# BerserkerMother/Video-Summarization

Measured on AMD Instinct MI355X. Metric: frames/sec scored (whole node), synthetic [B,T=1024,D=1024], higher is better.
Workload: dtype f32; 1 GPU; configs[2]: B=64 videos x T=1024 frames x D=1024 per GPU, scorer cfg M-A (heads 4, d_model 256, layers 4), logits + hidden state; global_batch=64, parallelism=videos sharded over 1 GPU(s), no all_gather of scores

## Files before the change

video-summarization_amd/csrc/vs_attention.hip:

```cpp
#include "vs_device.h"
#include "vs_kernels.h"

namespace {

template <int DH, int NKB, bool VARLEN = false>
__global__ __launch_bounds__(256, 2) void attn_fwd(
    const float *__restrict__ Q, const float *__restrict__ Kg, const float *__restrict__ Vg,
    const uint8_t *__restrict__ mask, float *__restrict__ out, int H, int T, float scale_log2e, int BH,
    const int *__restrict__ cu = nullptr, const int2 *__restrict__ work = nullptr, int Mtot = 0) {
    constexpr int KT = 32 * NKB, LD = DH + 4, NJ = DH / 8, ND = DH / 32;
    constexpr int F4 = KT * DH / 4 / 256;
    __shared__ __attribute__((aligned(16))) float Ks[KT * LD];
    __shared__ __attribute__((aligned(16))) float Vs[KT * LD];
    __shared__ float mb[KT];

    const int tid = threadIdx.x, lane = tid & 63, wave = tid >> 6;
    const int r = lane & 31, h = lane >> 5;
    int b, head, qt;
    size_t base, orow0;
    if constexpr (VARLEN) {
        const int2 wk = work[blockIdx.x];
        b = wk.x; qt = wk.y; head = blockIdx.y;
        const int c0 = cu[b];
        T = cu[b + 1] - c0;
// ... 750 lines not shown
        gload_m(KAHEAD);
        asm volatile("s_waitcnt vmcnt(0)" ::: "memory");
    } else {
#pragma unroll
        for (int u = 0; u < KAHEAD; ++u) {
            gload_k(u); gload_m(u);
            if (u < VAHEAD) gload_v(u);
#pragma unroll
            for (int i = 0; i < KPT; ++i) stage_k1(i, u % NBUF);
            if (u < VAHEAD) {
#pragma unroll
                for (int e = 0; e < 4; ++e) stage_v1(e, u % NBUF);
            }
            stage_m(u % NMB);
        }
        gload_k(KAHEAD); gload_m(KAHEAD); gload_v(VAHEAD);
    }
    __syncthreads();
    f32x16 sa[2], sb[2];
#pragma unroll
    for (int n = 0; n < 2; ++n)
#pragma unroll
        for (int t = 0; t < 16; ++t) { sa[n][t] = 0.f; sb[n][t] = 0.f; }
#pragma unroll
    for (int ks = 0; ks < NS; ++ks)
#pragma unroll
        for (int n = 0; n < 2; ++n) {
            u32x4 ka[NP];
            k_frag(0, ks, n, ka);
            static_for<NPROD>([&](auto prc) { mma_prod(prc, ka, qreg[ks], sa[n]); });
        }

    constexpr float CMARGIN = PREC == 2 ? -8.0f : 6.0f;
    (void)CMARGIN;
    u32x4 pf[2][2][NP];
    f16x2 pmaxh = {(_Float16)0.f, (_Float16)0.f};
    float cb_a = 0.f, cb_b = 0.f;
    auto rebase = [&](f32x16 (&sv)[2], float &cb, bool raise) __attribute__((always_inline)) {
        float mx = __builtin_fmaxf(__builtin_fmaxf(sv[0][0], sv[0][1]), sv[1][0]);
        mx = __builtin_fmaxf(mx, sv[1][1]);
#pragma unroll
        for (int t = 2; t < 16; t += 2) {
            mx = __builtin_fmaxf(__builtin_fmaxf(mx, sv[0][t]), sv[0][t + 1]);
            mx = __builtin_fmaxf(__builtin_fmaxf(mx, sv[1][t]), sv[1][t + 1]);
        }
        const float raw = pair_max(mx) + cb;
        float c_new = m_run;
        if ((raise || m_run == NEG_INF) && raw + CMARGIN > m_run) {
            const float cl = __builtin_fminf(__builtin_fmaxf(raw + CMARGIN, -32768.f), 32768.f);
            const unsigned b = __builtin_bit_cast(unsigned, cl);
            constexpr unsigned LOW = PREC == 2 ? 0x1FFFu : 0xFFFFu;
            c_new = __builtin_bit_cast(float, (cl >= 0.f ? b + LOW : b) & ~LOW);
            if (PREC == 1 && __builtin_fabsf(cl) >= 8192.f) c_new = __builtin_bit_cast(float, (b + 0x8000u) & ~LOW);
            if (PREC == 2 && __builtin_fabsf(c_new) < 0.0001220703125f) c_new = cl > 0.f ? 0.0001220703125f : 0.f;
        }
        const float u_new = (c_new == NEG_INF) ? 0.f : c_new;
        const float shift = cb - u_new;
        const float alpha = __builtin_amdgcn_exp2f(m_run - u_new);
#pragma unroll
        for (int n = 0; n < 2; ++n)
#pragma unroll
            for (int t = 0; t < 16; ++t) sv[n][t] += shift;
#pragma unroll
        for (int d = 0; d <= ND; ++d)
#pragma unroll
            for (int t = 0; t < 16; ++t) o[d][t] *= alpha;
        m_run = c_new;
        cb = u_new;
        unsigned pl[NP];
        pack(-u_new, 0.f, pl);
        nbias = h == 0 ? pl[0] : 0u;
    };
    auto p_pair = [&](auto kc, f32x16 (&sv)[2]) __attribute__((always_inline)) {
        constexpr int k = decltype(kc)::value, n = k / 8, ks = (k / 4) % 2, j = k % 4;
        unsigned pl[NP];
        pack(__builtin_amdgcn_exp2f(sv[n][8 * ks + 2 * j]), __builtin_amdgcn_exp2f(sv[n][8 * ks + 2 * j + 1]), pl);
#pragma unroll
        for (int p = 0; p < NP; ++p) pf[n][ks][p][j] = pl[p];
        if constexpr (PREC == 2) pmaxh = __builtin_elementwise_max(pmaxh, __builtin_bit_cast(f16x2, pl[0]));
    };
    float sm_mx = 0.f;
    f32x2 sm_mm = {0.f, 0.f};
    auto sm_unit_max = [&](auto uc, f32x16 (&sv)[2]) __attribute__((always_inline)) {
        constexpr int U = decltype(uc)::value;
        constexpr float THR = 8.0f;
        if constexpr (U == 0) {
            sm_mx = __builtin_fmaxf(__builtin_fmaxf(sv[0][0], sv[0][1]), sv[1][0]);
            sm_mx = __builtin_fmaxf(sm_mx, sv[1][1]);
        }
        if constexpr (U < 4) {
            constexpr int t0 = U == 0 ? 2 : 4 * U;
#pragma unroll
            for (int t = t0; t < 4 * U + 4; t += 2) {
                sm_mx = __builtin_fmaxf(__builtin_fmaxf(sm_mx, sv[0][t]), sv[0][t + 1]);
                sm_mx = __builtin_fmaxf(__builtin_fmaxf(sm_mx, sv[1][t]), sv[1][t + 1]);
            }
        }
        if constexpr (U == 4) {
            const float mx = pair_max(sm_mx);
            const bool raise = mx > m_run + THR || (m_run == NEG_INF && mx != NEG_INF);
            if (__builtin_expect(__any(raise), 0)) {
                const float m_new = raise ? mx : m_run;
                const float u_new = (m_new == NEG_INF) ? 0.f : m_new;
                const float alpha = __builtin_amdgcn_exp2f(m_run - u_new);
#pragma unroll
                for (int d = 0; d <= ND; ++d)
#pragma unroll
                    for (int t = 0; t < 16; ++t) o[d][t] *= alpha;
                m_run = m_new;
            }
            const float m_use = (m_run == NEG_INF) ? 0.f : m_run;
            sm_mm[0] = m_use; sm_mm[1] = m_use;
        }
        if constexpr (U >= 5 && U < 21) {
            constexpr int k = U - 5, n = k / 8, ks = (k / 4) % 2, j = k % 4;
            const f32x2 sx = {sv[n][8 * ks + 2 * j], sv[n][8 * ks + 2 * j + 1]};
            const f32x2 dv = sx - sm_mm;
            unsigned pl[NP];
            pack(__builtin_amdgcn_exp2f(dv[0]), __builtin_amdgcn_exp2f(dv[1]), pl);
#pragma unroll
            for (int p = 0; p < NP; ++p) pf[n][ks][p][j] = pl[p];
        }
    };
    auto sm_unit = [&](auto uc, f32x16 (&sv)[2], float &cb) __attribute__((always_inline)) {
        constexpr int U = decltype(uc)::value;
        if constexpr (!FOLD) { sm_unit_max(uc, sv); return; }
        if constexpr (U == 0) {
            const float u_run = (m_run == NEG_INF) ? 0.f : m_run;
            if (__builtin_expect(__any(cb != u_run || m_run == NEG_INF), 0)) rebase(sv, cb, false);
        }
        if constexpr (U >= 1 && U < 17) p_pair(std::integral_constant<int, U - 1>{}, sv);
        if constexpr (U == 17) {
            unsigned acc = 0u;
            bool hit;
            if constexpr (PREC == 2) {
                acc = __builtin_bit_cast(unsigned, pmaxh);
                hit = (acc & 0xFFFFu) >= 0x7800u || (acc >> 16) >= 0x7800u;
                pmaxh = f16x2{(_Float16)0.f, (_Float16)0.f};
            } else {
#pragma unroll
                for (int n = 0; n < 2; ++n)
#pragma unroll
                    for (int ks = 0; ks < 2; ++ks) acc |= (pf[n][ks][0][0] | pf[n][ks][0][1]) | (pf[n][ks][0][2] | pf[n][ks][0][3]);
                hit = (acc & 0x40004000u) != 0u;
            }
            if (__builtin_expect(__any(hit), 0)) {
                const unsigned hbit = hit ? 1u : 0u;
                auto pr = __builtin_amdgcn_permlane32_swap(hbit, hbit, false, false);
                rebase(sv, cb, (((unsigned)pr[0] | (unsigned)pr[1]) & 1u) != 0u);
                static_for<16>([&](auto kc) { p_pair(kc, sv); });
                if constexpr (PREC == 2) pmaxh = f16x2{(_Float16)0.f, (_Float16)0.f};
            }
        }
    };
    constexpr int NU = FOLD ? 18 : 21;
    constexpr bool FULLPF = PREC == 1 && DH <= 64;
    constexpr int NKF = FULLPF ? NS * 2 : 2, NVF = FULLPF ? 4 * ND : 2;
    constexpr int NBIAS = FOLD ? 2 : 0;
    constexpr int NSLOT_A = 2 * NS * NPROD + NBIAS, RA = (NU + NSLOT_A - 1) / NSLOT_A;
    constexpr int NSLOT_B = 4 * (ND * NPROD + NP);
    constexpr int NITEM = KPT + 4 + 2, SB = NSLOT_B / NITEM > 0 ? NSLOT_B / NITEM : 1;

    u32x4 abl_frag = {0u, 0u, 0u, 0u};
    if constexpr ((ABL & 16) != 0) abl_frag = *(const u32x4 *)&Kb[0][0][r * LDK + 8 * h];
    auto iteration = [&](int t, f32x16 (&s_in)[2], float &cb_in, f32x16 (&s_out)[2], float &cb_out) __attribute__((always_inline)) {
        const int cur = (ABL & 4) ? 0 : t % NBUF, nxt = (ABL & 4) ? 0 : (t + 1) % NBUF;
        if (mask != nullptr || (t + 1) * KT > T) {
            const float *mp = mb[t % NMB];
#pragma unroll
            for (int n = 0; n < 2; ++n)
#pragma unroll
                for (int g = 0; g < 4; ++g) {
                    const f32x4 bv = *(const f32x4 *)&mp[32 * n + 8 * g + 4 * h];
#pragma unroll
                    for (int e = 0; e < 4; ++e) s_in[n][4 * g + e] += bv[e];
                }
        }
        cb_out = (m_run == NEG_INF) ? 0.f : m_run;
        const u32x4 nb = {nbias, 0u, 0u, 0u};
        const f32x16 zero16 = {0.f, 0.f, 0.f, 0.f, 0.f, 0.f, 0.f, 0.f, 0.f, 0.f, 0.f, 0.f, 0.f, 0.f, 0.f, 0.f};
        u32x4 ka[NKF][NP], va[NVF][NP];
        if constexpr ((ABL & 16) != 0) {
#pragma unroll
            for (int g = 0; g < NKF; ++g)
#pragma unroll
                for (int p = 0; p < NP; ++p) ka[g][p] = abl_frag;
#pragma unroll
            for (int g = 0; g < NVF; ++g)
#pragma unroll
                for (int p = 0; p < NP; ++p) va[g][p] = abl_frag;
        } else
        if constexpr (FULLPF) {
#pragma unroll
            for (int g = 0; g < NS * 2; ++g) k_frag(nxt, g % NS, g / NS, ka[g]);
        } else {
            k_frag(nxt, 0, 0, ka[0]);
        }
        __builtin_amdgcn_sched_barrier(0);
        static_for<NSLOT_A>([&](auto ic) {
            constexpr int i = decltype(ic)::value, PERN = NS * NPROD, n = i < NBIAS ? i : (i - NBIAS) / PERN,
                          w = i < NBIAS ? 0 : 1 + (i - NBIAS) % PERN;
            if constexpr (w == 0) {
                s_out[n] = mma(ones_u, nb, zero16);
            } else {
                constexpr int ks = (w - 1) / NPROD, pr = (w - 1) % NPROD, g = n * NS + ks;
                if constexpr (!FOLD && w == 1) s_out[n] = zero16;
                if constexpr (!(ABL & 16) && !FULLPF && pr == 0 && g + 1 < NS * 2) k_frag(nxt, (g + 1) % NS, (g + 1) / NS, ka[(g + 1) & 1]);
                mma_prod(std::integral_constant<int, pr>{}, ka[FULLPF ? g : (g & 1)], qreg[ks], s_out[n]);
            }
            if constexpr (!(ABL & 16) && FULLPF && i >= NBIAS && i - NBIAS < NVF) {
                constexpr int f = i - NBIAS;
                v_frag(cur, f / ND / 2, (f / ND) % 2, f % ND, va[f]);
            }
            static_for<RA>([&](auto rc) {
                constexpr int U = i * RA + decltype(rc)::value;
                if constexpr (U < NU && !(ABL & 8)) sm_unit(std::integral_constant<int, U>{}, s_in, cb_in);
            });
            __builtin_amdgcn_sched_barrier(0);
        });
        lap(1);
        if constexpr (DMA) asm volatile("s_waitcnt vmcnt(0)" ::: "memory");
        if constexpr (STAG && !(ABL & 2)) { __syncthreads(); lap(3); }
        if constexpr (!FULLPF && !(ABL & 16)) v_frag(cur, 0, 0, 0, va[0]);
        __builtin_amdgcn_sched_barrier(0);
        static_for<NSLOT_B>([&](auto ic) {
            constexpr int i = decltype(ic)::value;
            constexpr int PER = ND * NPROD + NP;
            constexpr int g = i / PER, w = i % PER, n = g / 2, ks = g % 2;
            if constexpr (w < ND * NPROD) {
                constexpr int d = w / NPROD, pr = w % NPROD, f = g * ND + d;
                if constexpr (!(ABL & 16) && !FULLPF && pr == 0 && f + 1 < 4 * ND)
                    v_frag(cur, (f + 1) / ND / 2, ((f + 1) / ND) % 2, (f + 1) % ND, va[(f + 1) & 1]);
                mma_prod(std::integral_constant<int, pr>{}, va[FULLPF ? f : (f & 1)], pf[n][ks], o[d]);
            } else {
                constexpr int p = NP - 1 - (w - ND * NPROD);
                o[ND] = mma(ones_u, pf[n][ks][p], o[ND]);
            }
            if constexpr (DMA) {
                if constexpr (!(ABL & 1) && i == 0) dma_issue(t + KAHEAD, t + VAHEAD, true, true);
                if constexpr (!(ABL & 1) && i == 4) { stage_m((t + KAHEAD) % NMB); gload_m(t + KAHEAD + 1); }
            } else
            if constexpr (!(ABL & 1) && i % SB == SB - 1 && i / SB < NITEM) {
                constexpr int item = i / SB;
                if constexpr (item < KPT) stage_k1(item, (t + KAHEAD) % NBUF);
                else if constexpr (item < KPT + 4) stage_v1(item - KPT, (t + VAHEAD) % NBUF);
                else if constexpr (item == KPT + 4) { stage_m((t + KAHEAD) % NMB); }
                else { gload_k(t + KAHEAD + 1); gload_m(t + KAHEAD + 1); gload_v(t + VAHEAD + 1); }
            }
            __builtin_amdgcn_sched_barrier(0);
        });
        lap(2);
        if constexpr (!(ABL & 2)) __syncthreads();
        lap(3);
    };

    lap(0);
    const bool late = STAG && __builtin_amdgcn_readfirstlane(wave) >= NW / 2;
    if (late) __syncthreads();
    int t = 0;
    for (; t + 1 < ntiles; t += 2) {
        iteration(t, sa, cb_a, sb, cb_b);
        iteration(t + 1, sb, cb_b, sa, cb_a);
    }
    if (t < ntiles) iteration(t, sa, cb_a, sb, cb_b);
    if (STAG && !late) __syncthreads();

    const int q = q0 + r;
    if (q < T) {
        const float inv = 1.0f / o[ND][0];
        float *op = out + (orow0 + q) * (H * DH) + head * DH;
        h16 *op16 = (h16 *)out + (orow0 + q) * (H * DH) + head * DH;
#pragma unroll
        for (int d = 0; d < ND; ++d)
#pragma unroll
            for (int g = 0; g < 4; ++g) {
                f32x4 v;
#pragma unroll
                for (int e = 0; e < 4; ++e) v[e] = o[d][4 * g + e] * inv;
                if constexpr (IO16) {
                    u32x2 u; u[0] = pack_bf16(v[0], v[1]); u[1] = pack_bf16(v[2], v[3]);
                    *(u32x2 *)(op16 + 32 * d + 8 * g + 4 * h) = u;
                } else
                *(f32x4 *)(op + 32 * d + 8 * g + 4 * h) = v;
            }
    }
    if constexpr (DIAG != 0) {
        asm volatile("s_waitcnt vmcnt(0)" ::: "memory");
        lap(7);
        dg[8] = tl - tbeg; dg[10] = __builtin_amdgcn_s_memrealtime(); dg[11] = (unsigned long long)ntiles;
        if (diag != nullptr && lane == 0) {
            unsigned long long *o_ = diag + ((size_t)blockIdx.x * NW + wave) * 16;
#pragma unroll
            for (int i = 0; i < 12; ++i) o_[i] = dg[i];
        }
    }
}

template <int DH, bool HAS_MASK, int NW, bool VARLEN = false, int DIAG = 0>
__global__ __launch_bounds__(64 * NW, 2) void attn_fwd_pipe(
    const float *__restrict__ Q, const float *__restrict__ Kg, const float *__restrict__ Vg,
    const uint8_t *__restrict__ mask, float *__restrict__ out, int H, int T, float scale_log2e, int BH,
    const int *__restrict__ cu = nullptr, const int2 *__restrict__ work = nullptr, int Mtot = 0,
    unsigned long long *__restrict__ diag = nullptr) {
    unsigned long long dg[13] = {0ull, 0ull, 0ull, 0ull, 0ull, 0ull, 0ull, 0ull, 0ull, 0ull, 0ull, 0ull, 0ull}, tbeg = 0, tl = 0;
    if constexpr (DIAG != 0) { dg[9] = __builtin_amdgcn_s_memrealtime(); tbeg = vs_stamp(); tl = tbeg; }
    auto lap = [&](int slot) __attribute__((always_inline)) {
        if constexpr (DIAG != 0) { const unsigned long long t = vs_stamp(); dg[slot] += t - tl; tl = t; }
    };
    constexpr int KT = 64, LD = DH + 4, NJ = DH / 8, ND = DH / 32;
    constexpr int NT = 64 * NW;
    constexpr int F4 = KT * DH / 4 / NT;
    constexpr int TILE = KT * LD;
    constexpr float THR = 8.0f;
    __shared__ __attribute__((aligned(16))) float smem[4 * TILE + 2 * KT];
    float *mbs = smem + 4 * TILE;

    const int tid = threadIdx.x, lane = tid & 63, wave = tid >> 6;
    const int r = lane & 31, h = lane >> 5;
    int b, head, qt;
    size_t base, orow0;
    if constexpr (VARLEN) {
        const int2 wk = work[blockIdx.x];
        b = wk.x; qt = wk.y; head = blockIdx.y;
        const int c0 = cu[b];
        T = cu[b + 1] - c0;
        base = ((size_t)head * Mtot + c0) * DH;
        orow0 = (size_t)c0;
    } else {
        int bh;
        if (!attn_block_map((T + 32 * NW - 1) / (32 * NW), BH, bh, qt)) return;
        b = bh / H; head = bh - b * H;
        base = (size_t)bh * T * DH;
        orow0 = (size_t)b * T;
    }
    const int q0 = qt * (32 * NW) + 32 * wave;
    const float NEG_INF = -__builtin_inff();
    const int ntiles = (T + KT - 1) / KT;

    float qreg[4 * NJ];
    static_assert(4 * TILE >= NW * 32 * LD || NW == 8, "LDS corner per wave");
    float *wtp = smem + wave * (32 * LD);
    {
#pragma unroll
        for (int i = 0; i < DH / 8; ++i) {
            const int idx = lane + 64 * i;
            const int row = idx / (DH / 4), c4 = (idx % (DH / 4)) * 4;
            int qr = q0 + row; qr = qr < T ? qr : T - 1;
            *(f32x4 *)&wtp[row * LD + c4] = *(const f32x4 *)(Q + base + (size_t)qr * DH + c4);
        }
#pragma unroll
        for (int j = 0; j < NJ; ++j) {
            const f32x4 v = *(const f32x4 *)&wtp[r * LD + 8 * j + 4 * h];
#pragma unroll
            for (int s = 0; s < 4; ++s) qreg[4 * j + s] = v[s] * scale_log2e;
        }
    }
    lap(12);
    __syncthreads();
    f32x16 o[ND];
#pragma unroll
    for (int d = 0; d < ND; ++d)
#pragma unroll
        for (int t = 0; t < 16; ++t) o[d][t] = 0.f;
    float m_run = NEG_INF, l_run = 0.f;
    const float ones_a = h == 0 ? 1.0f : 0.0f;

    const __amdgpu_buffer_rsrc_t krs = __builtin_amdgcn_make_buffer_rsrc(
        const_cast<float *>(Kg + base), 0, T * DH * 4, 0x00020000);
    const __amdgpu_buffer_rsrc_t vrs = __builtin_amdgcn_make_buffer_rsrc(
        const_cast<float *>(Vg + base), 0, T * DH * 4, 0x00020000);
    int voff[F4];
#pragma unroll
    for (int i = 0; i < F4; ++i) {
        const int idx = tid + NT * i;
        voff[i] = ((idx / (DH / 4)) * DH + (idx % (DH / 4)) * 4) * 4;
    }
    f32x4 pk[F4], pv[F4];
    float pm = 0.f;
    auto gload_k = [&](int i, int tile) __attribute__((always_inline)) { pk[i] = __builtin_bit_cast(f32x4, __builtin_amdgcn_raw_buffer_load_b128(krs, voff[i], tile * (KT * DH * 4), 0)); };
    auto gload_v = [&](int i, int tile) __attribute__((always_inline)) { pv[i] = __builtin_bit_cast(f32x4, __builtin_amdgcn_raw_buffer_load_b128(vrs, voff[i], tile * (KT * DH * 4), 0)); };
    auto gload_m = [&](int tile) __attribute__((always_inline)) {
        const int key = tile * KT + (tid & (KT - 1));
        float pmv = key >= T ? NEG_INF : 0.f;
        if (HAS_MASK) pmv = mask[(size_t)b * T + (key < T ? key : T - 1)] != 0 ? NEG_INF : pmv;
        pm = pmv;
    };
    auto stage_k = [&](int i, int buf) __attribute__((always_inline)) {
        const int idx = tid + NT * i;
        *(f32x4 *)&smem[buf * 2 * TILE + (idx / (DH / 4)) * LD + (idx % (DH / 4)) * 4] = pk[i];
    };
    auto stage_v = [&](int i, int buf) __attribute__((always_inline)) {
        const int idx = tid + NT * i;
        *(f32x4 *)&smem[buf * 2 * TILE + TILE + (idx / (DH / 4)) * LD + (idx % (DH / 4)) * 4] = pv[i];
    };

    float sm_mx = 0.f, sm_psum = 0.f;
    float vreg[16 * ND];
    auto fixup = [&](f32x16 &sv, float m_bias, float raw_max) __attribute__((always_inline)) {
        const float m_new = (raw_max > m_run + THR || m_run == NEG_INF) ? fmaxf(m_run, raw_max) : m_run;
        const float u_new = (m_new == NEG_INF) ? 0.f : m_new;
        const float shift = m_bias - u_new;
        const float alpha = __builtin_amdgcn_exp2f(m_run - u_new);
#pragma unroll
        for (int t = 0; t < 16; ++t) sv[t] += shift;
#pragma unroll
        for (int d = 0; d < ND; ++d)
#pragma unroll
            for (int t = 0; t < 16; ++t) o[d][t] *= alpha;
        l_run *= alpha;
        m_run = m_new;
    };
    auto sm_unit = [&](auto uc, f32x16 &sv, float m_bias, const float *mb, auto masked_tag) __attribute__((always_inline)) {
        constexpr int U = decltype(uc)::value;
        constexpr bool MASKED = decltype(masked_tag)::value;
        if constexpr (MASKED && U < 4) {
            const f32x4 bv = *(const f32x4 *)(mb + 8 * U + 4 * h);
#pragma unroll
            for (int e = 0; e < 4; ++e) sv[4 * U + e] += bv[e];
        }
        if constexpr (U == 4) {
            sm_mx = fmaxf(fmaxf(sv[0], sv[1]), sv[2]);
#pragma unroll
            for (int t = 3; t < 15; t += 2) sm_mx = fmaxf(fmaxf(sm_mx, sv[t]), sv[t + 1]);
            sm_mx = fmaxf(sm_mx, sv[15]);
        }
        if constexpr (U == 5) {
            const float raw_max = pair_max(sm_mx) + m_bias;
            const float u_run = (m_run == NEG_INF) ? 0.f : m_run;
            const bool fix = (m_bias != u_run) || (raw_max > m_run + THR) || (m_run == NEG_INF && raw_max != NEG_INF);
            if (__builtin_expect(__any(fix), 0)) fixup(sv, m_bias, raw_max);
            sm_psum = 0.f;
        }
        if constexpr (U >= 8 && U < 16) {
            constexpr int k = U - 8;
#pragma unroll
            for (int e = 0; e < 2; ++e) {
                const float pe_ = __builtin_amdgcn_exp2f(sv[2 * k + e]);
                sv[2 * k + e] = pe_;
                sm_psum += pe_;
            }
        }
        if constexpr (U == 16) l_run += pair_sum(sm_psum);
    };
    auto half_step = [&](const float *Ksrc, int blk, f32x16 &s_out, float m_bias_out, f32x16 &s_in, float m_bias_in,
                         const float *mb, const float *Vsrc, int vblk, auto masked_tag, auto stage_tag, int nbuf, int ntile) __attribute__((always_inline)) {
        constexpr bool STAGE = decltype(stage_tag)::value;
        constexpr int NSLOT = 4 * NJ, R = 32 / NSLOT;
        static_assert(NSLOT == 16 * ND, "one V operand per MFMA slot");
        const float *kp = Ksrc + (32 * blk + r) * LD + 4 * h;
        const float *vp = Vsrc + (32 * vblk + 4 * h) * LD + r;
        f32x4 ka[2];
        ka[0] = *(const f32x4 *)kp;
        const f32x16 zero = {0.f, 0.f, 0.f, 0.f, 0.f, 0.f, 0.f, 0.f, 0.f, 0.f, 0.f, 0.f, 0.f, 0.f, 0.f, 0.f};
        s_out = MFMA32(ones_a, -m_bias_out, zero);
        __builtin_amdgcn_sched_barrier(0);
        static_for<NSLOT>([&](auto ic) {
            constexpr int i = decltype(ic)::value, j = i / 4, st = i % 4;
            if constexpr (st == 0 && j + 1 < NJ) ka[(j + 1) & 1] = *(const f32x4 *)(kp + 8 * (j + 1));
            s_out = MFMA32(ka[j & 1][st], qreg[4 * j + st], s_out);
            {
                constexpr int t = i / ND, d = i % ND;
                vreg[i] = vp[((t & 3) + 8 * (t >> 2)) * LD + 32 * d];
            }
            static_for<R>([&](auto rc) {
                constexpr int U = i * R + decltype(rc)::value;
                sm_unit(std::integral_constant<int, U>{}, s_in, m_bias_in, mb, masked_tag);
                if constexpr (STAGE) {
                    if constexpr (U < 2 * F4) { if constexpr (U % 2 == 0) stage_k(U / 2, nbuf); else stage_v(U / 2, nbuf); }
                    if constexpr (U == 2 * F4) mbs[nbuf * KT + (tid & (KT - 1))] = pm;
                    if constexpr (U >= 17 && U < 17 + 2 * F4) { if constexpr ((U - 17) % 2 == 0) gload_k((U - 17) / 2, ntile); else gload_v((U - 17) / 2, ntile); }
                    if constexpr (U == 17 + 2 * F4) gload_m(ntile);
                }
            });
            __builtin_amdgcn_sched_barrier(0);
        });
    };
    auto softmax_only = [&](f32x16 &sv, float m_bias, const float *mb, const float *Vsrc, int vblk, auto masked_tag) __attribute__((always_inline)) {
        const float *vp = Vsrc + (32 * vblk + 4 * h) * LD + r;
#pragma unroll
        for (int i = 0; i < 16 * ND; ++i) vreg[i] = vp[(((i / ND) & 3) + 8 * ((i / ND) >> 2)) * LD + 32 * (i % ND)];
        static_for<32>([&](auto uc) { sm_unit(uc, sv, m_bias, mb, masked_tag); });
    };
    auto pv_acc = [&](const f32x16 &p) __attribute__((always_inline)) {
#pragma unroll
        for (int t = 0; t < 16; ++t)
#pragma unroll
            for (int d = 0; d < ND; ++d) o[d] = MFMA32(vreg[ND * t + d], p[t], o[d]);
    };

#pragma unroll
    for (int i = 0; i < F4; ++i) { gload_k(i, 0); gload_v(i, 0); }
    gload_m(0);
#pragma unroll
    for (int i = 0; i < F4; ++i) { stage_k(i, 0); stage_v(i, 0); }
    mbs[tid & (KT - 1)] = pm;
    {
        const int t1 = ntiles > 1 ? 1 : 0;
#pragma unroll
        for (int i = 0; i < F4; ++i) { gload_k(i, t1); gload_v(i, t1); }
        gload_m(t1);
    }
    __syncthreads();
    f32x16 s_cur, s_nxt;
    float mb_cur = 0.f, mb_nxt = 0.f;
    {
        const float *kp = smem + r * LD + 4 * h;
#pragma unroll
        for (int t = 0; t < 16; ++t) s_cur[t] = 0.f;
#pragma unroll
        for (int j = 0; j < NJ; ++j) {
            const f32x4 ka = *(const f32x4 *)(kp + 8 * j);
#pragma unroll
            for (int st = 0; st < 4; ++st) s_cur = MFMA32(ka[st], qreg[4 * j + st], s_cur);
        }
    }

    auto tile_step = [&](int t, auto masked_tag, auto last_tag) __attribute__((always_inline)) {
        constexpr bool LAST = decltype(last_tag)::value;
        const int buf = t & 1;
        const float *Ks = smem + buf * 2 * TILE, *Vs = Ks + TILE;
        const float *Kn = smem + (buf ^ 1) * 2 * TILE;
        __syncthreads();
        lap(1);
        mb_nxt = (m_run == NEG_INF) ? 0.f : m_run;
        half_step(Ks, 1, s_nxt, mb_nxt, s_cur, mb_cur, mbs + buf * KT, Vs, 0, masked_tag, std::integral_constant<bool, !LAST>{},
                  buf ^ 1, t + 2 < ntiles ? t + 2 : ntiles - 1);
        lap(2);
        pv_acc(s_cur);
        lap(3);
        __syncthreads();
        lap(4);
        if constexpr (!LAST) {
            mb_cur = (m_run == NEG_INF) ? 0.f : m_run;
            half_step(Kn, 0, s_cur, mb_cur, s_nxt, mb_nxt, mbs + buf * KT + 32, Vs, 1, masked_tag, std::false_type{}, 0, 0);
        } else {
            softmax_only(s_nxt, mb_nxt, mbs + buf * KT + 32, Vs, 1, masked_tag);
        }
        lap(5);
        pv_acc(s_nxt);
        lap(6);
    };
    lap(0);
    for (int t = 0; t + 1 < ntiles; ++t) tile_step(t, std::integral_constant<bool, HAS_MASK>{}, std::false_type{});
    if (HAS_MASK || (T % KT) != 0) tile_step(ntiles - 1, std::true_type{}, std::true_type{});
    else                           tile_step(ntiles - 1, std::false_type{}, std::true_type{});

    __syncthreads();
    {
        const float inv = 1.0f / l_run;
#pragma unroll
        for (int d = 0; d < ND; ++d)
#pragma unroll
            for (int g = 0; g < 4; ++g) {
                f32x4 v;
#pragma unroll
                for (int e = 0; e < 4; ++e) v[e] = o[d][4 * g + e] * inv;
                *(f32x4 *)&wtp[r * LD + 32 * d + 8 * g + 4 * h] = v;
            }
        constexpr int LPR = DH / 4, RPI = 64 / LPR;
        const int orow = lane / LPR, oc4 = (lane % LPR) * 4;
#pragma unroll
        for (int p = 0; p < 32 / RPI; ++p) {
            const int rr = orow + RPI * p, q = q0 + rr;
            const f32x4 v = *(const f32x4 *)&wtp[rr * LD + oc4];
            if (q < T) *(f32x4 *)(out + (orow0 + q) * (H * DH) + head * DH + oc4) = v;
        }
    }
    if constexpr (DIAG != 0) {
        asm volatile("s_waitcnt vmcnt(0)" ::: "memory");
        lap(7);
        dg[8] = tl - tbeg; dg[10] = __builtin_amdgcn_s_memrealtime(); dg[11] = (unsigned long long)ntiles;
        dg[0] -= dg[12];
        if (diag != nullptr && lane == 0) {
            unsigned long long *o = diag + ((size_t)blockIdx.x * NW + wave) * 16;
#pragma unroll
            for (int i = 0; i < 13; ++i) o[i] = dg[i];
        }
    }
}

}

#ifdef VS_WITH_DIAG
int vsk_diag_attention(const float *q, const float *k, const float *v, float *out, int B, int H, int T, float scale,
                       unsigned long long *diag, hipStream_t st) {
    const int BH = B * H, nq = (T + 255) / 256;
    dim3 g(8 * ((BH + 7) / 8) * nq);
    hipLaunchKernelGGL((attn_fwd_pipe<64, false, 8, false, 1>), g, dim3(512), 0, st, q, k, v, nullptr, out, H, T,
                       scale * 1.4426950408889634f, BH, nullptr, nullptr, 0, diag);
    VSK_CHECK_LAUNCH();
    return (int)g.x;
}
int vsk_diag_attention_lp(const float *q, const float *k, const float *v, float *out, int B, int H, int T, float scale,
                          int prec, unsigned long long *diag, hipStream_t st) {
    const int BH = B * H, nq = (T + 255) / 256;
    dim3 g(8 * ((BH + 7) / 8) * nq);
    const float sl2 = scale * 1.4426950408889634f;
    if (prec >= 100) {
#define VSK_ABL(A_) case A_: hipLaunchKernelGGL((attn_fwd_lp_pipe<64, 8, 1, false, true, 0, A_>), g, dim3(512), 0, st, q, k, v, nullptr, out, H, T, sl2, BH, nullptr, nullptr, 0, nullptr); break;
        switch (prec - 100) {
            VSK_ABL(0) VSK_ABL(1) VSK_ABL(2) VSK_ABL(3) VSK_ABL(4) VSK_ABL(5) VSK_ABL(7) VSK_ABL(16) VSK_ABL(17) VSK_ABL(19)
            default: return -1;
        }
#undef VSK_ABL
        VSK_CHECK_LAUNCH();
        return (int)g.x;
    }
    if (prec == 1)
        hipLaunchKernelGGL((attn_fwd_lp_pipe<64, 8, 1, false, true, 1>), g, dim3(512), 0, st, q, k, v, nullptr, out, H, T, sl2, BH,
                           nullptr, nullptr, 0, diag);
    else
        hipLaunchKernelGGL((attn_fwd_lp_pipe<64, 8, 2, false, false, 1>), g, dim3(512), 0, st, q, k, v, nullptr, out, H, T, sl2, BH,
                           nullptr, nullptr, 0, diag);
    VSK_CHECK_LAUNCH();
    return (int)g.x;
}
#endif

float vsk_attention_qscale(float scale) { return scale * 1.4426950408889634f; }

int vsk_attention(const float *q, const float *k, const float *v, const uint8_t *mask, float *out,
                  int B, int H, int T, int dh, float scale, hipStream_t st) {
    const float sl2 = vsk_attention_qscale(scale);
    const int BH = B * H;
    dim3 grid(8 * ((BH + 7) / 8) * ((T + 127) / 128));
#ifdef VS_WITH_DIAG
    const bool legacy = vsk_options().attn_legacy != 0;
    if (dh == 32 && legacy)
        hipLaunchKernelGGL((attn_fwd<32, 2>), grid, dim3(256), 0, st, q, k, v, mask, out, H, T, sl2, BH);
    else if (dh == 64 && legacy)
        hipLaunchKernelGGL((attn_fwd<64, 2>), grid, dim3(256), 0, st, q, k, v, mask, out, H, T, sl2, BH);
    else
#endif
    if (dh == 32 || dh == 64) {
        const int r8 = (T + 255) / 256 * 256, r4 = (T + 127) / 128 * 128;
        const bool wide = !vsk_options().attn_nw4 && r8 * 100 <= r4 * 105;
        const int nq = wide ? r8 / 256 : r4 / 128;
        dim3 g(8 * ((BH + 7) / 8) * nq), blk(wide ? 512 : 256);
#define VSK_ATTN(DH_, MASK_, NW_) \
    hipLaunchKernelGGL((attn_fwd_pipe<DH_, MASK_, NW_, false>), g, blk, 0, st, q, k, v, mask, out, H, T, sl2, BH, nullptr, nullptr, 0, nullptr)
        if (dh == 32) {
            if (mask) { if (wide) VSK_ATTN(32, true, 8); else VSK_ATTN(32, true, 4); }
            else      { if (wide) VSK_ATTN(32, false, 8); else VSK_ATTN(32, false, 4); }
        } else {
            if (mask) { if (wide) VSK_ATTN(64, true, 8); else VSK_ATTN(64, true, 4); }
            else      { if (wide) VSK_ATTN(64, false, 8); else VSK_ATTN(64, false, 4); }
        }
#undef VSK_ATTN
    }
    else if (dh == 128)
        hipLaunchKernelGGL((attn_fwd<128, 1>), grid, dim3(256), 0, st, q, k, v, mask, out, H, T, sl2, BH);
    else
        return -1;
    VSK_CHECK_LAUNCH();
    return 0;
}

int vsk_attention_splitkv(const float *q, const float *k, const float *v, const uint8_t *mask, float *out,
                          int B, int H, int T, int dh, float scale, hipStream_t st) {
    const float sl2 = vsk_attention_qscale(scale);
    const dim3 grid(((T + 31) / 32) * B * H);
    if (dh == 64) hipLaunchKernelGGL((attn_fwd_splitkv<64>), grid, dim3(512), 0, st, q, k, v, mask, out, H, T, sl2, B * H);
    else if (dh == 128) hipLaunchKernelGGL((attn_fwd_splitkv<128>), grid, dim3(512), 0, st, q, k, v, mask, out, H, T, sl2, B * H);
    else if (dh == 32) hipLaunchKernelGGL((attn_fwd_splitkv<32>), grid, dim3(512), 0, st, q, k, v, mask, out, H, T, sl2, B * H);
    else return -1;
    VSK_CHECK_LAUNCH();
    return 0;
}

int vsk_attention_packed(const float *q, const float *k, const float *v, float *out, int H, int Mtot, int dh,
                         float scale, const int *cu, const int *work, int nwork, int nw, int prec, hipStream_t st) {
    const float sl2 = vsk_attention_qscale(scale);
    if (nwork <= 0) return 0;
    if (prec == (1 | VSK_STORE16) && dh == 64 && nw == 8 && vsk_options().attn_w64)
        return vsk_attention_bf16_w64_packed(q, k, v, out, H, Mtot, cu, work, nwork, st);
    dim3 grid(nwork, H);
    const int2 *wk = (const int2 *)work;
#define VSK_ATTN_PX(DH_, NW_) \
    hipLaunchKernelGGL((attn_fwd_pipe<DH_, false, NW_, true>), grid, dim3(64 * NW_), 0, st, q, k, v, nullptr, out, H, 0, sl2, 0, cu, wk, Mtot, nullptr)
#define VSK_ATTN_PE(DH_, NW_, P_) \
    hipLaunchKernelGGL((attn_fwd_lp_pipe<DH_, NW_, P_, true>), grid, dim3(64 * NW_), 0, st, q, k, v, nullptr, out, H, 0, sl2, 0, cu, wk, Mtot)
#define VSK_ATTN_P16(DH_, NW_) \
    hipLaunchKernelGGL((attn_fwd_lp_pipe<DH_, NW_, 1, true, true>), grid, dim3(64 * NW_), 0, st, q, k, v, nullptr, out, H, 0, sl2, 0, cu, wk, Mtot)
    if (prec == (1 | VSK_STORE16)) {
        if (dh == 64 && nw == 8) VSK_ATTN_P16(64, 8);
        else if (dh == 64 && nw == 4) VSK_ATTN_P16(64, 4);
        else if (dh == 32 && nw == 4) VSK_ATTN_P16(32, 4);
        else return -1;
    } else if (prec == 2) {
        if (dh == 64 && nw == 8) VSK_ATTN_PE(64, 8, 2);
        else if (dh == 64 && nw == 4) VSK_ATTN_PE(64, 4, 2);
        else if (dh == 32 && nw == 4) VSK_ATTN_PE(32, 4, 2);
        else return -1;
    } else if (prec == 1) {
        if (dh == 128 && nw == 8) VSK_ATTN_PE(128, 8, 1);
        else if (dh == 64 && nw == 8) VSK_ATTN_PE(64, 8, 1);
        else if (dh == 64 && nw == 4) VSK_ATTN_PE(64, 4, 1);
        else if (dh == 32 && nw == 4) VSK_ATTN_PE(32, 4, 1);
        else return -1;
    } else {
        if (dh == 128 && nw == 4)
            hipLaunchKernelGGL((attn_fwd<128, 1, true>), grid, dim3(256), 0, st, q, k, v, nullptr, out, H, 0, sl2, 0, cu, wk, Mtot);
        else if (dh == 64 && nw == 8) VSK_ATTN_PX(64, 8);
        else if (dh == 64 && nw == 4) VSK_ATTN_PX(64, 4);
        else if (dh == 32 && nw == 8) VSK_ATTN_PX(32, 8);
        else if (dh == 32 && nw == 4) VSK_ATTN_PX(32, 4);
        else return -1;
    }
#undef VSK_ATTN_PX
#undef VSK_ATTN_PE
#undef VSK_ATTN_P16
    VSK_CHECK_LAUNCH();
    return 0;
}

int vsk_attention_bf16(const float *q, const float *k, const float *v, const uint8_t *mask, float *out,
                       int B, int H, int T, int dh, float scale, int prec, hipStream_t st) {
    const float sl2 = vsk_attention_qscale(scale);
    const int BH = B * H;
    const int r8 = (T + 255) / 256 * 256, r4 = (T + 127) / 128 * 128;
    const bool wide = dh == 64 && !vsk_options().attn_nw4 && r8 * 100 <= r4 * 105;
    dim3 grid(8 * ((BH + 7) / 8) * (wide ? r8 / 256 : r4 / 128));
    const bool simple = vsk_options().attn_lp_simple != 0;
    if (dh == 128) {
        if (prec != 1 && prec != (1 | VSK_STORE16)) return -1;
        dim3 g128(8 * ((BH + 7) / 8) * (r8 / 256));
        if (prec == (1 | VSK_STORE16))
            hipLaunchKernelGGL((attn_fwd_lp_pipe<128, 8, 1, false, true>), g128, dim3(512), 0, st, q, k, v, mask, out, H, T, sl2, BH);
        else
        hipLaunchKernelGGL((attn_fwd_lp_pipe<128, 8, 1>), g128, dim3(512), 0, st, q, k, v, mask, out, H, T, sl2, BH);
        VSK_CHECK_LAUNCH();
        return 0;
    }
#define VSK_ATTN_LP(KERN_, P_)                                                                                           \
    if (dh == 64 && wide)                                                                                                \
        hipLaunchKernelGGL((KERN_<64, 8, P_>), grid, dim3(512), 0, st, q, k, v, mask, out, H, T, sl2, BH);               \
    else if (dh == 64)                                                                                                   \
        hipLaunchKernelGGL((KERN_<64, 4, P_>), grid, dim3(256), 0, st, q, k, v, mask, out, H, T, sl2, BH);               \
    else if (dh == 32)                                                                                                   \
        hipLaunchKernelGGL((KERN_<32, 4, P_>), grid, dim3(256), 0, st, q, k, v, mask, out, H, T, sl2, BH);               \
    else                                                                                                                 \
        return -1;
    if (prec == (1 | VSK_STORE16)) {
        if (dh == 64 && wide && vsk_options().attn_w64) {
            const int rc = vsk_attention_bf16_w64(q, k, v, mask, out, B, H, T, st);
            if (rc != -1) return rc;
        }
        if (dh == 64 && wide)
            hipLaunchKernelGGL((attn_fwd_lp_pipe<64, 8, 1, false, true>), grid, dim3(512), 0, st, q, k, v, mask, out, H, T, sl2, BH);
        else if (dh == 64)
            hipLaunchKernelGGL((attn_fwd_lp_pipe<64, 4, 1, false, true>), grid, dim3(256), 0, st, q, k, v, mask, out, H, T, sl2, BH);
        else if (dh == 32)
            hipLaunchKernelGGL((attn_fwd_lp_pipe<32, 4, 1, false, true>), grid, dim3(256), 0, st, q, k, v, mask, out, H, T, sl2, BH);
        else
            return -1;
    } else
    if (simple) { if (prec == 2) { VSK_ATTN_LP(attn_fwd_lp, 2) } else { VSK_ATTN_LP(attn_fwd_lp, 1) } }
    else        { if (prec == 2) { VSK_ATTN_LP(attn_fwd_lp_pipe, 2) } else { VSK_ATTN_LP(attn_fwd_lp_pipe, 1) } }
#undef VSK_ATTN_LP
    VSK_CHECK_LAUNCH();
    return 0;
}
```

Before: 11.99 million frames/s.

## Triple-buffer K/V tiles and add speculative fast-path softmax for unmasked tiles

For the 8-wave attention kernel, K/V shared-memory staging moves from double to triple buffering, with rotating buffer indices. This allows one of the two block barriers per tile to be dropped and the other moved earlier. Unmasked tiles now take a speculative softmax path that skips the per-block max reduction: it exponentiates against the running max and falls back to a full max/rescale path only when the partial sum overflows a threshold or a fix is forced. The cost is more shared memory per block, which may lower occupancy, plus an extra probability register vector.

```diff
diff --git a/video-summarization_amd/csrc/vs_attention.hip b/video-summarization_amd/csrc/vs_attention.hip
--- a/video-summarization_amd/csrc/vs_attention.hip
+++ b/video-summarization_amd/csrc/vs_attention.hip
@@ -1076,7 +1076,7 @@
     const uint8_t *__restrict__ mask, float *__restrict__ out, int H, int T, float scale_log2e, int BH,
     const int *__restrict__ cu = nullptr, const int2 *__restrict__ work = nullptr, int Mtot = 0,
     unsigned long long *__restrict__ diag = nullptr) {
-    unsigned long long dg[13] = {0ull, 0ull, 0ull, 0ull, 0ull, 0ull, 0ull, 0ull, 0ull, 0ull, 0ull, 0ull, 0ull}, tbeg = 0, tl = 0;
+    unsigned long long dg[14] = {0ull, 0ull, 0ull, 0ull, 0ull, 0ull, 0ull, 0ull, 0ull, 0ull, 0ull, 0ull, 0ull, 0ull}, tbeg = 0, tl = 0;
     if constexpr (DIAG != 0) { dg[9] = __builtin_amdgcn_s_memrealtime(); tbeg = vs_stamp(); tl = tbeg; }
     auto lap = [&](int slot) __attribute__((always_inline)) {
         if constexpr (DIAG != 0) { const unsigned long long t = vs_stamp(); dg[slot] += t - tl; tl = t; }
@@ -1086,8 +1086,9 @@
     constexpr int F4 = KT * DH / 4 / NT;
     constexpr int TILE = KT * LD;
     constexpr float THR = 8.0f;
-    __shared__ __attribute__((aligned(16))) float smem[4 * TILE + 2 * KT];
-    float *mbs = smem + 4 * TILE;
+    constexpr int NBUF = NW == 8 ? 3 : 2;
+    __shared__ __attribute__((aligned(16))) float smem[2 * NBUF * TILE + NBUF * KT];
+    float *mbs = smem + 2 * NBUF * TILE;
 
     const int tid = threadIdx.x, lane = tid & 63, wave = tid >> 6;
     const int r = lane & 31, h = lane >> 5;
@@ -1136,7 +1137,8 @@
     for (int d = 0; d < ND; ++d)
 #pragma unroll
         for (int t = 0; t < 16; ++t) o[d][t] = 0.f;
-    float m_run = NEG_INF, l_run = 0.f;
+    float m_run = NEG_INF, u_run = 0.f, l_run = 0.f;
+    auto m_use = [&]() __attribute__((always_inline)) { return HAS_MASK ? ((m_run == NEG_INF) ? 0.f : m_run) : u_run; };
     const float ones_a = h == 0 ? 1.0f : 0.0f;
 
     const __amdgpu_buffer_rsrc_t krs = __builtin_amdgcn_make_buffer_rsrc(
@@ -1183,10 +1185,46 @@
             for (int t = 0; t < 16; ++t) o[d][t] *= alpha;
         l_run *= alpha;
         m_run = m_new;
-    };
-    auto sm_unit = [&](auto uc, f32x16 &sv, float m_bias, const float *mb, auto masked_tag) __attribute__((always_inline)) {
+        u_run = u_new;
+    };
+    unsigned long long sm_force = ~0ull;
+    auto sm_slow = [&](f32x16 &sv, f32x16 &p, float m_bias) __attribute__((always_inline)) {
+        if constexpr (DIAG != 0) dg[13] += 1;
+        float mx = fmaxf(fmaxf(sv[0], sv[1]), sv[2]);
+#pragma unroll
+        for (int t = 3; t < 15; t += 2) mx = fmaxf(fmaxf(mx, sv[t]), sv[t + 1]);
+        mx = fmaxf(mx, sv[15]);
+        const float raw_max = pair_max(mx) + m_bias;
+        const bool fix = (m_bias != m_use()) || (raw_max > m_run + THR) || (m_run == NEG_INF && raw_max != NEG_INF);
+        if (__any(fix)) { fixup(sv, m_bias, raw_max); sm_force = ~0ull; }
+        sm_psum = 0.f;
+#pragma unroll
+        for (int t = 0; t < 16; ++t) {
+            p[t] = __builtin_amdgcn_exp2f(sv[t]);
+            sm_psum += p[t];
+        }
+    };
+    auto sm_unit = [&](auto uc, f32x16 &sv, f32x16 &p, float m_bias, const float *mb, auto masked_tag) __attribute__((always_inline)) {
         constexpr int U = decltype(uc)::value;
         constexpr bool MASKED = decltype(masked_tag)::value;
+        if constexpr (!MASKED) {
+            if constexpr (U == 8) sm_psum = 0.f;
+            if constexpr (U >= 8 && U < 16) {
+#pragma unroll
+                for (int e = 0; e < 2; ++e) {
+                    const int t = 2 * (U - 8) + e;
+                    p[t] = __builtin_amdgcn_exp2f(sv[t]);
+                    sm_psum += p[t];
+                }
+            }
+            if constexpr (U == 16) {
+                const unsigned long long slow = sm_force | __builtin_amdgcn_ballot_w64(!(sm_psum < 255.0f));
+                sm_force = 0ull;
+                if (__builtin_expect(slow != 0ull, 0)) sm_slow(sv, p, m_bias);
+                l_run += pair_sum(sm_psum);
+            }
+            return;
+        }
         if constexpr (MASKED && U < 4) {
             const f32x4 bv = *(const f32x4 *)(mb + 8 * U + 4 * h);
 #pragma unroll
@@ -1200,8 +1238,8 @@
         }
         if constexpr (U == 5) {
             const float raw_max = pair_max(sm_mx) + m_bias;
-            const float u_run = (m_run == NEG_INF) ? 0.f : m_run;
-            const bool fix = (m_bias != u_run) || (raw_max > m_run + THR) || (m_run == NEG_INF && raw_max != NEG_INF);
+            const float u_use = (m_run == NEG_INF) ? 0.f : m_run;
+            const bool fix = (m_bias != u_use) || (raw_max > m_run + THR) || (m_run == NEG_INF && raw_max != NEG_INF);
             if (__builtin_expect(__any(fix), 0)) fixup(sv, m_bias, raw_max);
             sm_psum = 0.f;
         }
@@ -1216,7 +1254,7 @@
         }
         if constexpr (U == 16) l_run += pair_sum(sm_psum);
     };
-    auto half_step = [&](const float *Ksrc, int blk, f32x16 &s_out, float m_bias_out, f32x16 &s_in, float m_bias_in,
+    auto half_step = [&](const float *Ksrc, int blk, f32x16 &s_out, float m_bias_out, f32x16 &s_in, f32x16 &p_in, float m_bias_in,
                          const float *mb, const float *Vsrc, int vblk, auto masked_tag, auto stage_tag, int nbuf, int ntile) __attribute__((always_inline)) {
         constexpr bool STAGE = decltype(stage_tag)::value;
         constexpr int NSLOT = 4 * NJ, R = 32 / NSLOT;
@@ -1238,7 +1276,7 @@
             }
             static_for<R>([&](auto rc) {
                 constexpr int U = i * R + decltype(rc)::value;
-                sm_unit(std::integral_constant<int, U>{}, s_in, m_bias_in, mb, masked_tag);
+                sm_unit(std::integral_constant<int, U>{}, s_in, p_in, m_bias_in, mb, masked_tag);
                 if constexpr (STAGE) {
                     if constexpr (U < 2 * F4) { if constexpr (U % 2 == 0) stage_k(U / 2, nbuf); else stage_v(U / 2, nbuf); }
                     if constexpr (U == 2 * F4) mbs[nbuf * KT + (tid & (KT - 1))] = pm;
@@ -1249,11 +1287,11 @@
             __builtin_amdgcn_sched_barrier(0);
         });
     };
-    auto softmax_only = [&](f32x16 &sv, float m_bias, const float *mb, const float *Vsrc, int vblk, auto masked_tag) __attribute__((always_inline)) {
+    auto softmax_only = [&](f32x16 &sv, f32x16 &p, float m_bias, const float *mb, const float *Vsrc, int vblk, auto masked_tag) __attribute__((always_inline)) {
         const float *vp = Vsrc + (32 * vblk + 4 * h) * LD + r;
 #pragma unroll
         for (int i = 0; i < 16 * ND; ++i) vreg[i] = vp[(((i / ND) & 3) + 8 * ((i / ND) >> 2)) * LD + 32 * (i % ND)];
-        static_for<32>([&](auto uc) { sm_unit(uc, sv, m_bias, mb, masked_tag); });
+        static_for<32>([&](auto uc) { sm_unit(uc, sv, p, m_bias, mb, masked_tag); });
     };
     auto pv_acc = [&](const f32x16 &p) __attribute__((always_inline)) {
 #pragma unroll
@@ -1289,35 +1327,45 @@
         }
     }
 
-    auto tile_step = [&](int t, auto masked_tag, auto last_tag) __attribute__((always_inline)) {
+    f32x16 p_blk;
+    auto tile_step = [&](int t, int bc, int bn, auto masked_tag, auto last_tag) __attribute__((always_inline)) {
         constexpr bool LAST = decltype(last_tag)::value;
-        const int buf = t & 1;
-        const float *Ks = smem + buf * 2 * TILE, *Vs = Ks + TILE;
-        const float *Kn = smem + (buf ^ 1) * 2 * TILE;
-        __syncthreads();
-        lap(1);
-        mb_nxt = (m_run == NEG_INF) ? 0.f : m_run;
-        half_step(Ks, 1, s_nxt, mb_nxt, s_cur, mb_cur, mbs + buf * KT, Vs, 0, masked_tag, std::integral_constant<bool, !LAST>{},
-                  buf ^ 1, t + 2 < ntiles ? t + 2 : ntiles - 1);
+        constexpr bool BAR_EARLY = NBUF == 3;
+        constexpr bool INPLACE = decltype(masked_tag)::value;
+        const float *Ks = smem + bc * 2 * TILE, *Vs = Ks + TILE;
+        const float *Kn = smem + bn * 2 * TILE;
+        if constexpr (NBUF == 2) {
+            __syncthreads();
+            lap(1);
+        }
+        mb_nxt = m_use();
+        half_step(Ks, 1, s_nxt, mb_nxt, s_cur, p_blk, mb_cur, mbs + bc * KT, Vs, 0, masked_tag, std::integral_constant<bool, !LAST>{},
+                  bn, t + 2 < ntiles ? t + 2 : ntiles - 1);
         lap(2);
-        pv_acc(s_cur);
+        if constexpr (BAR_EARLY) { __syncthreads(); lap(4); }
+        if constexpr (INPLACE) pv_acc(s_cur); else pv_acc(p_blk);
         lap(3);
-        __syncthreads();
-        lap(4);
+        if constexpr (!BAR_EARLY) { __syncthreads(); lap(4); }
         if constexpr (!LAST) {
-            mb_cur = (m_run == NEG_INF) ? 0.f : m_run;
-            half_step(Kn, 0, s_cur, mb_cur, s_nxt, mb_nxt, mbs + buf * KT + 32, Vs, 1, masked_tag, std::false_type{}, 0, 0);
+            mb_cur = m_use();
+            half_step(Kn, 0, s_cur, mb_cur, s_nxt, p_blk, mb_nxt, mbs + bc * KT + 32, Vs, 1, masked_tag, std::false_type{}, 0, 0);
         } else {
-            softmax_only(s_nxt, mb_nxt, mbs + buf * KT + 32, Vs, 1, masked_tag);
+            softmax_only(s_nxt, p_blk, mb_nxt, mbs + bc * KT + 32, Vs, 1, masked_tag);
         }
         lap(5);
-        pv_acc(s_nxt);
+        if constexpr (INPLACE) pv_acc(s_nxt); else pv_acc(p_blk);
         lap(6);
     };
     lap(0);
-    for (int t = 0; t + 1 < ntiles; ++t) tile_step(t, std::integral_constant<bool, HAS_MASK>{}, std::false_type{});
-    if (HAS_MASK || (T % KT) != 0) tile_step(ntiles - 1, std::true_type{}, std::true_type{});
-    else                           tile_step(ntiles - 1, std::false_type{}, std::true_type{});
+    int bc = 0, bn = 1, bf = 2;
+    for (int t = 0; t + 1 < ntiles; ++t) {
+        tile_step(t, bc, bn, std::integral_constant<bool, HAS_MASK>{}, std::false_type{});
+        const int b0 = bc;
+        bc = bn;
+        if constexpr (NBUF == 3) { bn = bf; bf = b0; } else { bn = b0; }
+    }
+    if (HAS_MASK || (T % KT) != 0) tile_step(ntiles - 1, bc, bn, std::true_type{}, std::true_type{});
+    else                           tile_step(ntiles - 1, bc, bn, std::false_type{}, std::true_type{});
 
     __syncthreads();
     {
@@ -1348,7 +1396,7 @@
         if (diag != nullptr && lane == 0) {
             unsigned long long *o = diag + ((size_t)blockIdx.x * NW + wave) * 16;
 #pragma unroll
-            for (int i = 0; i < 13; ++i) o[i] = dg[i];
+            for (int i = 0; i < 14; ++i) o[i] = dg[i];
         }
     }
 }
```

Result: no change. 12.08 million frames/s (median of 6 runs) (+0.8%).
